# acerbilab/vbmc

Hardware: AMD Instinct MI355X
Metric: ELBO+grad evals/sec (Ns=1e4, K=50, D=10, N=400) (higher is better)
Workload: dtype f64; 1 GPU; BASELINE configs[2]: D=10 N=400 K=50 Ns=10000/component S=20, R=64 restarts batched per GPU per step, value+gradient, beta=0, no variance; restarts_per_gpu=64, parallelism=one GPU

## Files before the change

### vbmc_amd/csrc/entropy_mfma.h

```cpp
#pragma once
#include <type_traits>

#include "device_math.h"
#include "elbo_types.h"
#include "exp2_tab1k.h"
#include "logjoint_body.h"

typedef double mf4 __attribute__((ext_vector_type(4)));
struct EntTileAny { static constexpr bool rt = false, val = true; };
struct EntTileFull { static constexpr bool rt = false, val = false; };
struct EntTilePartial { static constexpr bool rt = false, val = true; };
#define VBMC_ENT_SPLIT(KT_, QS_, TL_, HV_) ((HV_) == 1)

#ifdef VBMC_INSTRUMENT
#define VBMC_DBG_WAVES 32768
__device__ unsigned long long g_ent_dbg[6 * VBMC_DBG_WAVES];
#endif

#define VBMC_STAG_FOR(KT_, QS_, TL_) ((KT_) == 1 || (KT_) == 4 || ((KT_) == 2 && (QS_) >= 6) || ((KT_) == 3 && (QS_) <= ((TL_) ? 5 : 8)))



constexpr bool ent_c2_for(int KT, int QS, int TL, int HV) {
  if (HV == 1) {
    if (KT == 2) return !(TL == 1 && QS >= 6);
    if (KT == 3) return QS <= 5 || (TL == 0 && QS != 7) || (TL == 1 && QS == 7);
    if (KT == 4) return QS >= 5;
    return true;
  }
  if (HV == 2) {
    if (KT == 2) return TL != 2;
    if (KT == 3) return !((TL == 1 && (QS == 5 || QS == 6)) || (TL == 2 && QS == 6));
    return true;
  }
  if (KT == 2) return !((TL == 1 && QS >= 6) || (TL == 2 && QS >= 5));
  if (KT == 3) return !(TL == 1 && QS == 7);
  return QS != 5;
}
constexpr bool ent_gp2_for(int KT, int QS, int TL, int HV) { return !(HV == 1 && KT == 1 && TL == 0 && QS <= 3); }

template <int HV>
__device__ __forceinline__ void ent_sync() {
  __builtin_amdgcn_fence(__ATOMIC_RELEASE, "wavefront");
  __builtin_amdgcn_wave_barrier();
  __builtin_amdgcn_fence(__ATOMIC_ACQUIRE, "wavefront");
}
template <int HV>
__device__ __forceinline__ void ent_sync_wg() {
  if (HV == 1) ent_sync<1>();
  else __syncthreads();
}

template <int QS, int KT, bool GRAD, bool SPARSE, int HV = 1, int TL = 0, bool CO = false, bool EM = true, bool WALK = false>
#define VBMC_ENT_EO(HV_) true
#define VBMC_ENT_ONE_WAVE(KT_, QS_, TL_, HV_) \
  (((HV_) == 1 && (KT_) == 4 && (QS_) >= 5) || ((HV_) == 1 && (KT_) == 3 && (QS_) >= 8) || ((HV_) == 4 && (KT_) == 4 && (QS_) >= 6) || \
   ((HV_) == 4 && (KT_) == 3 && (QS_) >= 9))
#define VBMC_ENT_WAVES(KT_, QS_, TL_, HV_) \
  (VBMC_ENT_ONE_WAVE(KT_, QS_, TL_, HV_) ? 1 : ((((KT_) <= 2 && (QS_) <= 4) && !((KT_) == 2 && (TL_) == 2 && (HV_) == 1)) ? 3 : 2))
__device__ __forceinline__ void ent_mfma_segment(const EntArgs& a, const int c, const int j, const int r, const int t0, const int t1,
                                                 const int pdone, const int ptot) {
  static_assert(!CO || (HV == 1 && QS <= 8 && !SPARSE), "the log-joint role exists for single-wave dense kernels at D <= 30");
  static_assert(!WALK || (HV == 1 && !CO), "the walk exists for single-wave workgroups without the log-joint role");
  static_assert(KT <= 4 && (HV == 1 || HV == 2 || HV == 4 || HV == 8), "larger mixtures are split over the waves of a workgroup (HV = 2, 4; round 5: 8, K <= 512)");
  static_assert(TL == 0 || ((TL == 1 || TL == 2) && !SPARSE), "the component tail (one or two values per lane) exists for the dense kernels only");
  constexpr int TLN = TL > 0 ? TL : 1;
  constexpr bool SP = SPARSE;
  constexpr int DP = 4 * QS;
  constexpr int NPV = (4 * QS + 15) / 16;
  constexpr int QL = QS;
  __shared__ double Et[16 * DP];
  constexpr bool GP2 = GRAD && ent_gp2_for(KT, QS, TL, HV);
  __shared__ double RQ_all[HV][GP2 ? 32 : 16];
  __shared__ double BND_all[HV][SPARSE ? KT * 16 * 3 : 1];
  constexpr int YXN = NPV * 4 * WAVE;
  constexpr bool EO = VBMC_ENT_EO(HV);
  constexpr bool YXSB = HV > 1 && EO;
  constexpr bool US = EO;
  constexpr bool VBL = GRAD && HV == 1 && (KT >= 3 || NPV >= 2);
  __shared__ double VBS_all[HV][VBL ? KT * 4 * NPV * WAVE : 1];
  constexpr bool C2 = EO && !SPARSE && ent_c2_for(KT, QS, TL, HV);
#define ENT_CI(kt_, rr_) (16 * (kt_) + 4 * (rr_) + lg)
  __shared__ __attribute__((aligned(16))) double SCP_all[HV][C2 ? KT * 16 * 2 : 2];
  __shared__ double BTL_all[HV][TL ? 4 * TL * DP : 1];
  constexpr bool NML = HV > 1 && EO;
  __shared__ double NMS_all[HV][NML ? KT * 4 * WAVE : 1];
#ifdef VBMC_INSTRUMENT
  const unsigned long long wckE = wall_clock64();
#endif
  int tid_ = threadIdx.x;
  if (WALK) asm volatile("" : "+v"(tid_));
  const int tid = tid_, wv = tid >> 6, hv = HV == 1 ? 0 : wv, lane = tid & 63;
  const int li = lane & 15, lg = lane >> 4;
  int D_ = a.D, K_ = a.K;
  const double *entp_ = a.entp, *vpd_ = a.vpd;
  double* part_ = a.part;
  if (WALK) asm volatile("" : "+s"(D_), "+s"(K_), "+s"(entp_), "+s"(vpd_), "+s"(part_));
  const int D = D_, K = K_;
  double* RQ = RQ_all[wv];
  double* NMS = NMS_all[wv];
  double* BND = BND_all[hv];
  double* VBS = VBS_all[hv];
  double* BTL = BTL_all[hv];
  double* SCP = SCP_all[hv];
  const int Kh = (K + HV - 1) / HV;
  const int kbase = hv * Kh;
  const int Kw = min(K, kbase + Kh) - kbase;
  const int PSg = D + ENTP_EXTRA;
  extern __shared__ double PB[];
  double* const TAB = PB;
  double* const YX = PB + VB_EXP_TAB1K_N;
  constexpr int NTH0 = WAVE * HV;
  constexpr int NTB0 = (VB_EXP_TAB1K_N + NTH0 - 1) / NTH0;
  double tt[NTB0];
#pragma unroll
  for (int u = 0; u < NTB0; ++u) tt[u] = c_exp2_tab1k[min(tid + u * NTH0, VB_EXP_TAB1K_N - 1)];
  const double sigj = vpd_[(size_t)r * VpLayout{D, K}.stride() + VpLayout{D, K}.sigma() + j];
  {
    const double* gsrc = entp_ + (size_t)r * K * PSg;
    constexpr int NT = WAVE * HV;
    const int n = K * PSg;
    int idx = tid;
    for (; idx + 7 * NT < n; idx += 8 * NT) {
      double t8[8];
#pragma unroll
      for (int u = 0; u < 8; ++u) t8[u] = gsrc[idx + u * NT];
#pragma unroll
      for (int u = 0; u < 8; ++u) PB[idx + u * NT] = t8[u];
    }
    {
      double t8[8];
#pragma unroll
      for (int u = 0; u < 8; ++u) t8[u] = (idx + u * NT < n) ? gsrc[idx + u * NT] : 0.0;
#pragma unroll
      for (int u = 0; u < 8; ++u) if (idx + u * NT < n) PB[idx + u * NT] = t8[u];
    }
  }
  __syncthreads();
  const double* gp = PB;
  const double* pj = gp + (size_t)j * PSg;
  const double cKj = pj[D + 1];
  const double hj_neg = 0.5 / (sigj * sigj);
  const int nr_last = TL ? 4 : max(1, min(4, (Kw - 16 * (KT - 1) + 3) >> 2));
  constexpr unsigned FULL_MASK = (1u << KT) - 1u;
  const double logwj = SPARSE ? log(pj[D + 2]) : 0.0;

  constexpr double ESC = VB_EXP_TAB1K_SCALE;
  double SA[KT][QL];
  double SC[KT];
  double VB[VBL ? 1 : KT][4][NPV];
  double WF[KT][4];
#pragma unroll
  for (int kt = 0; kt < KT; ++kt) {
    const int k = 16 * kt + li;
    const bool kv = k < Kw;
    const double* pk = gp + (size_t)(kv ? kbase + k : 0) * PSg;
    double h = pk[D];
    double m2 = 0.0;
    for (int d = 0; d < D; ++d) { double t = pk[d] - pj[d]; m2 = fma(t, t, m2); }
    if (SPARSE && lg == 0) {
      BND[(16 * kt + li) * 3 + 0] = sqrt(m2);
      BND[(16 * kt + li) * 3 + 1] = kv ? pk[D + 1] - cKj : -1.0e30;
      BND[(16 * kt + li) * 3 + 2] = h;
    }
#pragma unroll
    for (int q = 0; q < QL; ++q) {
      const int cc = 4 * q + lg;
      if (EO) {
        double sav = (kv && cc < D) ? ESC * (-2.0 * h * (pk[cc] - pj[cc])) : 0.0;
        if (C2) {
          if (cc == D) sav = kv ? ESC * (h + hj_neg) : 0.0;
          if (cc == D + 1) sav = ESC * (kv ? fma(h, m2, pk[D + 1]) - cKj : -1.0e6);
        }
        SA[kt][q] = sav;
      } else {
        double v;
        if (!kv) v = (cc == D + 1) ? -1.0e6 : 0.0;
        else if (cc < D) v = -2.0 * h * (pk[cc] - pj[cc]);
        else if (cc == D) v = h + hj_neg;
        else if (cc == D + 1) v = fma(h, m2, pk[D + 1]) - cKj;
        else v = 0.0;
        SA[kt][q] = ESC * v;
      }
    }
    SC[kt] = ESC * (!kv ? (lg == 1 ? -1.0e6 : 0.0)
                        : (lg == 0 ? h + hj_neg : (lg == 1 ? fma(h, m2, pk[D + 1]) - cKj : 0.0)));
    if (C2 && lg < 2) SCP[(16 * kt + li) * 2 + lg] = 2.0 * SC[kt];
#pragma unroll
    for (int rr = 0; rr < 4; ++rr) {
      const int k2 = ENT_CI(kt, rr);
      const bool kv2 = k2 < Kw;
      const double* p2 = gp + (size_t)(kv2 ? kbase + k2 : 0) * PSg;
      if (GRAD) {
#pragma unroll
        for (int pv = 0; pv < NPV; ++pv) {
          const int col = 16 * pv + li;
          double v = 0.0;
          if (kv2) {
            if (col == 0) v = p2[D + 2];
            else if (col == 1) v = p2[D + 3];
            else if (col < 2 + D) v = p2[D + 3] * (p2[col - 2] - pj[col - 2]);
          }
          if (VBL) VBS[((kt * 4 + rr) * NPV + pv) * WAVE + lane] = v;
          else VB[VBL ? 0 : kt][rr][pv] = v;
        }
      } else {
        WF[kt][rr] = kv2 ? p2[D + 2] : 0.0;
      }
    }
  }

  double tC0[TLN], tC1[TLN], VBt[TLN][NPV], WFt[TLN], Wt[TLN];
#pragma unroll
  for (int u = 0; u < TLN; ++u) {
    tC0[u] = 0.0; tC1[u] = 0.0; WFt[u] = 0.0; Wt[u] = 0.0;
#pragma unroll
    for (int pv = 0; pv < NPV; ++pv) VBt[u][pv] = 0.0;
  }
  if (TL) {
#pragma unroll
    for (int u = 0; u < TLN; ++u) {
      const int tq = 4 * u + lg;
      const int kq = 16 * KT + tq;
      const bool kvq = kq < Kw;
      const double* pq = gp + (size_t)(kvq ? kbase + kq : 0) * PSg;
      const double h = pq[D];
      double m2 = 0.0;
      for (int d = 0; d < D; ++d) { double t = pq[d] - pj[d]; m2 = fma(t, t, m2); }
      tC0[u] = kvq ? ESC * (h + hj_neg) : 0.0;
      tC1[u] = ESC * (kvq ? fma(h, m2, pq[D + 1]) - cKj : -1.0e6);
      for (int d = li; d < DP; d += 16) BTL[tq * DP + d] = (kvq && d < D) ? ESC * (-2.0 * h * (pq[d] - pj[d])) : 0.0;
      if (GRAD) {
#pragma unroll
        for (int pv = 0; pv < NPV; ++pv) {
          const int col = 16 * pv + li;
          double v = 0.0;
          if (kvq) {
            if (col == 0) v = pq[D + 2];
            else if (col == 1) v = pq[D + 3];
            else if (col < 2 + D) v = pq[D + 3] * (pq[col - 2] - pj[col - 2]);
          }
          VBt[u][pv] = v;
        }
      } else {
        WFt[u] = kvq ? pq[D + 2] : 0.0;
      }
    }
  }

  __syncthreads();
  {
#pragma unroll
    for (int u = 0; u < NTB0; ++u) if (VB_EXP_TAB1K_N % NTH0 == 0 || tid + u * NTH0 < VB_EXP_TAB1K_N) TAB[tid + u * NTH0] = tt[u];
  }
  __syncthreads();

#define SAV(kt_, q_) SA[kt_][q_]
  constexpr int VBR = (VBL && NPV == 1 && HV == 1 && KT == 3 && !CO) ? ((EM && QS <= 4) ? (TL == 2 ? 4 : 10) : 12) : 0;
  double VBreg[VBR > 0 ? VBR : 1];
#pragma unroll
  for (int u = 0; u < VBR; ++u) VBreg[u] = VBS[u * WAVE + lane];
#define VBV(kt_, rr_, pv_) (VBL ? (((kt_) * 4 + (rr_)) * NPV + (pv_) < VBR ? VBreg[(((kt_) * 4 + (rr_)) * NPV + (pv_)) < VBR ? (((kt_) * 4 + (rr_)) * NPV + (pv_)) : 0] : VBS[(((kt_) * 4 + (rr_)) * NPV + (pv_)) * WAVE + lane]) : VB[VBL ? 0 : (kt_)][rr_][pv_])
  double accH = 0.0, accG[NPV], accLG[NPV];
  double pm = 1.0;
  int pe = 0, pcnt = 0;
  double Wacc[KT][4];
#pragma unroll
  for (int pv = 0; pv < NPV; ++pv) { accG[pv] = 0.0; accLG[pv] = 0.0; }
#pragma unroll
  for (int kt = 0; kt < KT; ++kt)
#pragma unroll
    for (int rr = 0; rr < 4; ++rr) Wacc[kt][rr] = 0.0;

#ifdef VBMC_INSTRUMENT
  const unsigned long long wck0 = wall_clock64();
#endif
  const int ntile = (a.Mh + 15) >> 4;
  const double sfm0 = lg == 0 ? 1.0 : 0.0, sfm1 = lg == 1 ? 1.0 : 0.0;
  const int emask = (4 * (QS - 1) + lg < D) ? -1 : 0;
  const int emask2 = (QS >= 2 && 4 * (QS - 2) + lg < D) ? -1 : 0;
  const double* epsr = a.eps ? a.eps + (size_t)r * a.eps_stride_r + (size_t)j * a.Mh * D : nullptr;
  constexpr bool EPF = EM && HV == 1 && QS <= 4 && KT <= 3 && !SPARSE;
  double epre[EPF ? QS : 1];
  auto eps_fetch = [&](const int tile) {
#pragma unroll
    for (int u = 0; u < (EPF ? QS : 0); ++u) {
      const int idx = lane + u * WAVE, i = idx / DP, d = idx - i * DP;
      double v = 0.0;
      if (tile < t1 && d < D && tile * 16 + i < a.Mh) v = epsr[(size_t)(tile * 16 + i) * D + d];
      epre[u] = v;
    }
  };
  if (EPF && epsr) eps_fetch(t0);
  if (!epsr && (HV == 1 || hv == 0))
    for (int idx = lane; idx < 16 * DP; idx += WAVE) Et[idx] = 0.0;
  const int evm1 = emask, evm2 = emask2;
  const double c2u1 = (4 * (QS - 1) + lg == D) ? 1.0 : 0.0, c2o1 = (4 * (QS - 1) + lg == D + 1) ? 1.0 : 0.0;
  const double c2u2 = (QS >= 2 && 4 * (QS - 2) + lg == D) ? 1.0 : 0.0;

  auto tile_body = [&](const int tile, auto pkind) __attribute__((always_inline)) {
    using PK = decltype(pkind);
    const int b0 = tile * 16;
    ent_sync_wg<HV>();
    if (HV > 1 && hv != 0) {
    } else if (EPF && epsr) {
#pragma unroll
      for (int u = 0; u < (EPF ? QS : 0); ++u) Et[lane + u * WAVE] = US ? sigj * epre[u] : epre[u];
      eps_fetch(tile + 1);
    } else if (epsr) {
      for (int idx = lane; idx < 16 * DP; idx += WAVE) {
        const int i = idx / DP, d = idx - i * DP;
        Et[idx] = (d < D && b0 + i < a.Mh) ? (US ? sigj * epsr[(size_t)(b0 + i) * D + d] : epsr[(size_t)(b0 + i) * D + d]) : 0.0;
      }
    } else {
      unsigned long long seed_t = a.seed;
      if (WALK) asm volatile("" : "+s"(seed_t));
#pragma unroll
      for (int q = lg; q < QS; q += 4) {
        double z4[4] = {0.0, 0.0, 0.0, 0.0};
#define VBMC_RNG_CALL_FOR(KT_, QS_, TL_, HV_) ((HV_) == 2 && (((KT_) == 2 && (TL_) == 2 && (QS_) == 5) || ((KT_) == 3 && (TL_) == 0 && (QS_) == 7)))
        if constexpr (!VBMC_RNG_CALL_FOR(KT, QS, TL, HV)) {
        if (q < (D + 3) / 4) { const vb_d4 zz = vb_normal4i(seed_t, (unsigned)(b0 + li), (unsigned)j, (unsigned)(a.r0 + r * a.rstride), (unsigned)q); z4[0] = zz[0]; z4[1] = zz[1]; z4[2] = zz[2]; z4[3] = zz[3]; }
        } else {
        if (q < (D + 3) / 4) vb_normal4(seed_t, (unsigned)(b0 + li), (unsigned)j, (unsigned)(a.r0 + r * a.rstride), (unsigned)q, z4);
        }
#undef VBMC_RNG_CALL_FOR
        if (q < (D + 3) / 4) {
#pragma unroll
        for (int t = 0; t < 4; ++t) Et[li * DP + 4 * q + t] = US ? sigj * z4[t] : z4[t];
        }
      }
    }
    ent_sync_wg<HV>();
    double ev[QS];
    double e2 = 0.0;
#pragma unroll
    for (int q = 0; q < QS; ++q) {
      ev[q] = Et[li * DP + 4 * q + lg];
      if (q == QS - 1) ev[q] = __hiloint2double(__double2hiint(ev[q]) & evm1, __double2loint(ev[q]) & evm1);
      if (QS >= 2 && q == QS - 2) ev[q] = __hiloint2double(__double2hiint(ev[q]) & evm2, __double2loint(ev[q]) & evm2);
      e2 = fma(ev[q], ev[q], e2);
    }
    e2 = xor_sum16(e2);
    e2 = xor_sum32(e2);
    double shift = US ? fma(-e2, hj_neg, cKj) : cKj - 0.5 * e2;
    const double u2 = US ? e2 : sigj * sigj * e2;
    if (US && SPARSE) e2 *= 2.0 * hj_neg;
    constexpr bool partial = PK::val;
    const bool svalid = b0 + li < a.Mh;
    if (partial) shift = svalid ? shift : 0.0;
    unsigned act = FULL_MASK;
    if (SPARSE) {
      double e2m = e2;
      e2m = fmax(e2m, __shfl_xor(e2m, 1, 64)); e2m = fmax(e2m, __shfl_xor(e2m, 2, 64));
      e2m = fmax(e2m, __shfl_xor(e2m, 4, 64)); e2m = fmax(e2m, __shfl_xor(e2m, 8, 64));
      const double umax = sigj * sqrt(e2m);
      const double own = 0.5 * e2m - logwj;
      act = 0u;
#pragma unroll
      for (int kt = 0; kt < KT; ++kt) {
        const double* bk = BND + (16 * kt + li) * 3;
        const double t = fmax(0.0, bk[0] - umax);
        const double bnd = fma(bk[2] * t, t, bk[1]) + own;
        if (__any(bnd > -a.cutoff)) act |= 1u << kt;
      }
    }

    mf4 n[KT], nm[(EO && !NML) ? KT : 1];
    if (EO) {
      const double sfc = fma(u2, sfm0, sfm1);
      double sfl[QL];
#pragma unroll
      for (int q = 0; q < QL; ++q) sfl[q] = US ? ev[q] : ev[q] * sigj;
      if (C2) {
        sfl[QL - 1] = fma(u2, c2u1, sfl[QL - 1] + c2o1);
        if (QS >= 2) sfl[QL >= 2 ? QL - 2 : 0] = fma(u2, c2u2, sfl[QL >= 2 ? QL - 2 : 0]);
      }
#pragma unroll
      for (int kt = 0; kt < KT; ++kt) {
        n[kt] = (mf4){0.0, 0.0, 0.0, 0.0};
        if (!NML) nm[(EO && !NML) ? kt : 0] = (mf4){0.0, 0.0, 0.0, 0.0};
        if (C2) {
#pragma unroll
          for (int q = 0; q < QL; ++q) n[kt] = __builtin_amdgcn_mfma_f64_16x16x4f64(SAV(kt, q), sfl[q], n[kt], 0, 0, 0);
          mf4 e2nd;
#pragma unroll
          for (int rr = 0; rr < 4; ++rr) {
            const double2 pr = *reinterpret_cast<const double2*>(SCP + ENT_CI(kt, rr) * 2);
            e2nd[rr] = fma(pr.x, u2, pr.y) - n[kt][rr];
          }
          if (NML) {
#pragma unroll
            for (int rr = 0; rr < 4; ++rr) NMS[(kt * 4 + rr) * WAVE + lane] = e2nd[rr];
          } else {
            nm[(EO && !NML) ? kt : 0] = e2nd;
          }
        } else
        if (!SP || ((act >> kt) & 1u)) {
          const mf4 cacc = __builtin_amdgcn_mfma_f64_16x16x4f64(SC[kt], sfc, n[kt], 0, 0, 0);
          n[kt] = cacc;
#pragma unroll
          for (int q = 0; q < QL; ++q)
            n[kt] = __builtin_amdgcn_mfma_f64_16x16x4f64(SAV(kt, q), sfl[q], n[kt], 0, 0, 0);
          if (NML) {
            const mf4 e2nd = 2.0 * cacc - n[kt];
#pragma unroll
            for (int rr = 0; rr < 4; ++rr) NMS[(kt * 4 + rr) * WAVE + lane] = e2nd[rr];
          } else {
            nm[(EO && !NML) ? kt : 0] = 2.0 * cacc - n[kt];
          }
        }
      }
    }

    double ntl[TLN], ntm[TLN];
#pragma unroll
    for (int u = 0; u < TLN; ++u) { ntl[u] = 0.0; ntm[u] = 0.0; }
    if (TL) {
#pragma unroll
      for (int u = 0; u < TLN; ++u) {
        double lt = 0.0;
#pragma unroll
        for (int d = 0; d < DP; ++d) lt = fma(BTL[(4 * u + lg) * DP + d], Et[li * DP + d], lt);
        if (!US) lt *= sigj;
        const double ct = fma(tC0[u], u2, tC1[u]);
        ntl[u] = ct + lt;
        ntm[u] = ct - lt;
      }
    }

    auto exps = [&](mf4 (&x)[KT], auto k0c, auto k1c) {
      constexpr int k0 = decltype(k0c)::value, k1 = decltype(k1c)::value;
#pragma unroll
      for (int kt = k0; kt < k1; ++kt) {
        if (kt < KT - 1) {
          if (!SP || ((act >> kt) & 1u)) x[kt] = vb_exp_tab1k4<VB_EXP_TAB1K_QUAD>(x[kt], TAB);
          else x[kt] = (mf4){0.0, 0.0, 0.0, 0.0};
        } else if (SP && !((act >> (KT - 1)) & 1u)) {
          x[KT - 1] = (mf4){0.0, 0.0, 0.0, 0.0};
        } else if (nr_last == 4) {
          x[KT - 1] = vb_exp_tab1k4<VB_EXP_TAB1K_QUAD>(x[KT - 1], TAB);
        } else {
          mf4 t = x[KT - 1];
          x[KT - 1] = (mf4){0.0, 0.0, 0.0, 0.0};
          x[KT - 1][0] = vb_exp_tab1k<VB_EXP_TAB1K_QUAD>(t[0], TAB);
          if (nr_last > 1) x[KT - 1][1] = vb_exp_tab1k<VB_EXP_TAB1K_QUAD>(t[1], TAB);
          if (nr_last > 2) x[KT - 1][2] = vb_exp_tab1k<VB_EXP_TAB1K_QUAD>(t[2], TAB);
        }
      }
    };
    auto texp = [&](double (&t)[TLN]) {
      if (TL) {
#pragma unroll
        for (int u = 0; u < TLN; ++u) t[u] = vb_exp_tab1k<VB_EXP_TAB1K_QUAD>(t[u], TAB);
      }
    };
    auto pvstep = [&](mf4 (&x)[KT], mf4 (&Y)[NPV], int sg, const double (&tn)[TLN]) {
      constexpr bool TWO = NPV == 1 && KT <= 2;
      mf4 Y2s[TWO ? NPV : 1];
      mf4 (&Y2)[TWO ? NPV : 1] = Y2s;
#pragma unroll
      for (int pv = 0; pv < NPV; ++pv) { Y[pv] = (mf4){0.0, 0.0, 0.0, 0.0}; if (TWO) Y2[pv] = (mf4){0.0, 0.0, 0.0, 0.0}; }
#pragma unroll
      for (int kt = 0; kt < KT - 1; ++kt) {
        if (SP && !((act >> kt) & 1u)) continue;
#pragma unroll
        for (int pv = 0; pv < NPV; ++pv) {
          mf4& Yb = TWO ? Y2[TWO ? pv : 0] : Y[pv];
          Y[pv] = __builtin_amdgcn_mfma_f64_16x16x4f64(x[kt][0], VBV(kt, 0, pv), Y[pv], 0, 0, 0);
          Yb = __builtin_amdgcn_mfma_f64_16x16x4f64(x[kt][1], VBV(kt, 1, pv), Yb, 0, 0, 0);
          Y[pv] = __builtin_amdgcn_mfma_f64_16x16x4f64(x[kt][2], VBV(kt, 2, pv), Y[pv], 0, 0, 0);
          Yb = __builtin_amdgcn_mfma_f64_16x16x4f64(x[kt][3], VBV(kt, 3, pv), Yb, 0, 0, 0);
        }
      }
#pragma unroll
      for (int pv = 0; pv < NPV; ++pv) {
        mf4& Yb = TWO ? Y2[TWO ? pv : 0] : Y[pv];
        if (SP && !((act >> (KT - 1)) & 1u)) { if (TWO) Y[pv] += Yb; continue; }
        Y[pv] = __builtin_amdgcn_mfma_f64_16x16x4f64(x[KT - 1][0], VBV(KT - 1, 0, pv), Y[pv], 0, 0, 0);
        if (nr_last > 1) Yb = __builtin_amdgcn_mfma_f64_16x16x4f64(x[KT - 1][1], VBV(KT - 1, 1, pv), Yb, 0, 0, 0);
        if (nr_last > 2) Y[pv] = __builtin_amdgcn_mfma_f64_16x16x4f64(x[KT - 1][2], VBV(KT - 1, 2, pv), Y[pv], 0, 0, 0);
        if (nr_last > 3) Yb = __builtin_amdgcn_mfma_f64_16x16x4f64(x[KT - 1][3], VBV(KT - 1, 3, pv), Yb, 0, 0, 0);
        if (TL) {
#pragma unroll
          for (int u = 0; u < TLN; ++u) Y[pv] = __builtin_amdgcn_mfma_f64_16x16x4f64(tn[u], VBt[u][pv], Y[pv], 0, 0, 0);
        }
        if (TWO) Y[pv] += Yb;
      }
      if (HV > 1) {
        if (YXSB && sg == 1) __syncthreads();
#pragma unroll
        for (int pv = 0; pv < NPV; ++pv)
#pragma unroll
          for (int rr = 0; rr < 4; ++rr) YX[((YXSB ? 0 : sg) * HV + hv) * YXN + (pv * 4 + rr) * WAVE + lane] = Y[pv][rr];
        __syncthreads();
#pragma unroll
        for (int pv = 0; pv < NPV; ++pv)
#pragma unroll
          for (int rr = 0; rr < 4; ++rr) {
            double t = YX[((YXSB ? 0 : sg) * HV + 0) * YXN + (pv * 4 + rr) * WAVE + lane];
#pragma unroll
            for (int w = 1; w < HV; ++w) t += YX[((YXSB ? 0 : sg) * HV + w) * YXN + (pv * 4 + rr) * WAVE + lane];
            Y[pv][rr] = t;
          }
      }
    };
    auto put_q = [&](mf4 (&Y)[NPV]) {
      if (GP2 ? li < 2 : li == 0) {
#pragma unroll
        for (int rr = 0; rr < 4; ++rr) RQ[(GP2 ? 16 * li : 0) + lg + 4 * rr] = Y[0][rr];
      }
      ent_sync<HV>();
    };
    double arq = 0.0;
    constexpr bool TQ = GP2 && US && NPV == 1 && HV == 1 && EO && KT == 3 && QS <= 3 && !CO && !EM && VBMC_STAG_FOR(KT, QS, TL);
    double tq[TQ ? 4 : 1];
    auto get_rq = [&]() -> double {
      double qs_ = RQ[li];
      double rqs = vb_rcp(qs_);
      if (partial) {
        qs_ = svalid ? qs_ : 1.0;
        rqs = svalid ? rqs : 0.0;
      }
      if (GP2) arq = RQ[GP2 ? 16 + li : 0] * rqs;
      pm *= __builtin_amdgcn_frexp_mant(qs_);
      pe += __builtin_amdgcn_frexp_exp(qs_);
      accH += shift;
      return rqs;
    };
    auto wacc = [&](mf4 (&x)[KT], double rqs, const double (&tn)[TLN]) {
      if (TL) {
#pragma unroll
        for (int u = 0; u < TLN; ++u) Wt[u] = fma(tn[u], rqs, Wt[u]);
      }
#pragma unroll
      for (int kt = 0; kt < KT; ++kt) {
        if (SP && !((act >> kt) & 1u)) continue;
#pragma unroll
        for (int rr = 0; rr < 4; ++rr) Wacc[kt][rr] = fma(x[kt][rr], rqs, Wacc[kt][rr]);
      }
    };
    auto put_rq = [&](double rqs) {
      ent_sync<HV>();
      if (lg == 0) { RQ[li] = rqs; if (GP2) RQ[GP2 ? 16 + li : 0] = arq; }
      ent_sync<HV>();
    };
    auto gradpieces = [&](mf4 (&Y)[NPV], double ssig, auto sgc) {
      constexpr int SG = decltype(sgc)::value;
      if constexpr (GP2) {
#pragma unroll
        for (int rr = 0; rr < 4; ++rr) {
          const int i = lg + 4 * rr;
          const double rq = RQ[i], ar = RQ[GP2 ? 16 + i : 0];
#pragma unroll
          for (int pv = 0; pv < NPV; ++pv) {
            if (HV > 1 && (pv % HV) != hv) continue;
            const int d = min(max(16 * pv + li - 2, 0), DP - 1);
            double tv;
            if (TQ) { if (SG >= 0) tq[TQ ? rr : 0] = Et[i * DP + d]; tv = tq[TQ ? rr : 0]; }
            else tv = Et[i * DP + d];
            const double t = (US && SG > 0) ? tv : ((US && SG < 0) ? -tv : ssig * tv);
            const double gd = fma(t, ar, -(Y[pv][rr] * rq));
            accG[pv] += gd;
            accLG[pv] = fma(t, gd, accLG[pv]);
          }
        }
        ent_sync<HV>();
        return;
      }
      const int base = lane & 48;
#pragma unroll
      for (int rr = 0; rr < 4; ++rr) {
        const int i = lg + 4 * rr;
        const double Av = __shfl(Y[0][rr], base | 1, 64);
        const double rq = RQ[i];
#pragma unroll
        for (int pv = 0; pv < NPV; ++pv) {
          if (HV > 1 && (pv % HV) != hv) continue;
          const int d = 16 * pv + li - 2;
          if (d >= 0 && d < D) {
            const double t = (US && SG > 0) ? Et[i * DP + d] : ((US && SG < 0) ? -Et[i * DP + d] : ssig * Et[i * DP + d]);
            const double gd = (t * Av - Y[pv][rr]) * rq;
            accG[pv] += gd;
            accLG[pv] = fma(t, gd, accLG[pv]);
          }
        }
      }
      ent_sync<HV>();
    };
    auto fold = [&]() {
      if (++pcnt == 256) {
        pe += __builtin_amdgcn_frexp_exp(pm);
        pm = __builtin_amdgcn_frexp_mant(pm);
        pcnt = 0;
      }
    };
    using I0 = std::integral_constant<int, 0>;
    using IH = std::integral_constant<int, (KT + 1) / 2>;
    using IK = std::integral_constant<int, KT>;

    if constexpr (EO && GRAD && HV == 1 && VBMC_STAG_FOR(KT, QS, TL)) {
      mf4 Y[NPV];
      exps(n, I0{}, IK{});
      texp(ntl);
      pvstep(n, Y, 0, ntl);
      put_q(Y);
      exps(nm, I0{}, IH{});
      const double rqs = get_rq();
      put_rq(rqs);
      exps(nm, IH{}, IK{});
      texp(ntm);
      wacc(n, rqs, ntl);
      gradpieces(Y, sigj, std::integral_constant<int, 1>{});
      fold();
      pvstep(nm, Y, 1, ntm);
      put_q(Y);
      const double rqs2 = get_rq();
      wacc(nm, rqs2, ntm);
      put_rq(rqs2);
      gradpieces(Y, -sigj, std::integral_constant<int, -1>{});
      fold();
    } else {
      int sg = 0;
      double ssig = US ? 1.0 : sigj;
#pragma unroll 1
      for (;;) {
        if (!EO) {
          double sf[QS];
#pragma unroll
          for (int q = 0; q < QS; ++q) {
            const int cc = 4 * q + lg;
            constexpr bool EVREG = KT <= 3 && QS <= 7;
            sf[q] = (cc < D) ? ssig * (EVREG ? ev[q] : Et[li * DP + 4 * q + lg]) : ((cc == D) ? u2 : ((cc == D + 1) ? 1.0 : 0.0));
          }
#pragma unroll
          for (int kt = 0; kt < KT; ++kt) {
            n[kt] = (mf4){0.0, 0.0, 0.0, 0.0};
#pragma unroll
            for (int q = 0; q < QS; ++q) n[kt] = __builtin_amdgcn_mfma_f64_16x16x4f64(SA[kt][q], sf[q], n[kt], 0, 0, 0);
          }
        }
        exps(n, I0{}, IK{});
        texp(ntl);
        if (GRAD) {
          mf4 Y[NPV];
          pvstep(n, Y, sg, ntl);
          put_q(Y);
          const double rqs = get_rq();
          wacc(n, rqs, ntl);
          put_rq(rqs);
          gradpieces(Y, ssig, std::integral_constant<int, 0>{});
        } else {
          double qp = 0.0;
#pragma unroll
          for (int kt = 0; kt < KT; ++kt)
#pragma unroll
            for (int rr = 0; rr < 4; ++rr) qp = fma(WF[kt][rr], n[kt][rr], qp);
          if (TL) {
#pragma unroll
            for (int u = 0; u < TLN; ++u) qp = fma(WFt[u], ntl[u], qp);
          }
          qp += __shfl_xor(qp, 16, 64);
          qp += __shfl_xor(qp, 32, 64);
          if (HV > 1) {
            if (YXSB && sg == 1) __syncthreads();
            YX[((YXSB ? 0 : sg) * HV + hv) * YXN + lane] = qp;
            __syncthreads();
            qp = YX[((YXSB ? 0 : sg) * HV + 0) * YXN + lane];
#pragma unroll
            for (int w = 1; w < HV; ++w) qp += YX[((YXSB ? 0 : sg) * HV + w) * YXN + lane];
          }
          double qs_ = qp;
          if (partial) qs_ = svalid ? qp : 1.0;
          pm *= __builtin_amdgcn_frexp_mant(qs_);
          pe += __builtin_amdgcn_frexp_exp(qs_);
          accH += shift;
        }
        fold();
        if (sg) break;
        sg = 1;
        ssig = US ? -1.0 : -sigj;
        if (EO) {
#pragma unroll
          for (int kt = 0; kt < KT; ++kt) {
            if (NML) {
#pragma unroll
              for (int rr = 0; rr < 4; ++rr) n[kt][rr] = NMS[(kt * 4 + rr) * WAVE + lane];
            } else {
              n[kt] = nm[(EO && !NML) ? kt : 0];
            }
          }
        }
#pragma unroll
        for (int u = 0; u < TLN; ++u) ntl[u] = ntm[u];
      }
    }
  };
  if constexpr (VBMC_ENT_SPLIT(KT, QS, TL, HV)) {
    const int tf = min(t1, a.Mh >> 4);
    constexpr bool PRIO = CO ? QS <= 4 : VBMC_ENT_WAVES(KT, QS, TL, HV) > 1;
    const bool pr = PRIO && a.prio != 0;
    const int q1 = pr ? t0 + (ptot + 3) / 4 - pdone : -1, q2 = pr ? t0 + (ptot + 1) / 2 - pdone : -1, q3 = pr ? t0 + (3 * ptot + 3) / 4 - pdone : -1;
    if (pr && pdone == 0) __builtin_amdgcn_s_setprio(3);
    for (int tile = t0; tile < tf; ++tile) {
      if (tile == q1) __builtin_amdgcn_s_setprio(2);
      if (tile == q2) __builtin_amdgcn_s_setprio(1);
      if (tile == q3) __builtin_amdgcn_s_setprio(0);
      tile_body(tile, EntTileFull{});
    }
    if (tf < t1) tile_body(tf, EntTilePartial{});
  } else {
    for (int tile = t0; tile < t1; ++tile) tile_body(tile, EntTileAny{});
  }
#ifdef VBMC_INSTRUMENT
  const unsigned long long wck1 = wall_clock64();
#endif
  if (WALK) accH += vb_log_pos(pm, &pe) + 0.693147180559945309417 * (double)pe;
  else accH += log(pm) + 0.693147180559945309417 * (double)pe;
  if (lg != 0) accH = 0.0;

  double* o = part_ + (((size_t)r * K + j) * a.C + c) * a.ncol;
  accH = wave_sum(accH);
  if (lane == 0 && hv == 0) o[0] = accH;
  if (GRAD) {
    double sgsum = 0.0;
#pragma unroll
    for (int pv = 0; pv < NPV; ++pv) {
      double g = accG[pv], lgd = accLG[pv] / sigj;
      g += __shfl_xor(g, 16, 64); g += __shfl_xor(g, 32, 64);
      lgd += __shfl_xor(lgd, 16, 64); lgd += __shfl_xor(lgd, 32, 64);
      const int d = 16 * pv + li - 2;
      const bool dv = d >= 0 && d < D;
      const bool mine = HV == 1 || (pv % HV) == hv;
      if (dv && lg == 0 && mine) { o[1 + d] = g; o[2 + D + d] = lgd; }
      sgsum += (dv && lg == 0 && mine) ? lgd : 0.0;
    }
    sgsum = wave_sum(sgsum);
    if (HV > 1) {
      __syncthreads();
      if (lane == 0) YX[hv * YXN] = sgsum;
      __syncthreads();
      sgsum = YX[0];
#pragma unroll
      for (int w = 1; w < HV; ++w) sgsum += YX[w * YXN];
    }
    if (lane == 0 && hv == 0) o[1 + D] = sgsum;
#pragma unroll
    for (int kt = 0; kt < KT; ++kt)
#pragma unroll
      for (int rr = 0; rr < 4; ++rr) {
        double wv = Wacc[kt][rr];
        wv += __shfl_xor(wv, 1, 64); wv += __shfl_xor(wv, 2, 64);
        wv += __shfl_xor(wv, 4, 64); wv += __shfl_xor(wv, 8, 64);
        const int k = ENT_CI(kt, rr);
        if (li == 0 && k < Kw) o[2 + 2 * D + kbase + k] = wv;
      }
    if (TL) {
#pragma unroll
      for (int u = 0; u < TLN; ++u) {
        double wv = Wt[u];
        wv += __shfl_xor(wv, 1, 64); wv += __shfl_xor(wv, 2, 64);
        wv += __shfl_xor(wv, 4, 64); wv += __shfl_xor(wv, 8, 64);
        const int k = 16 * KT + 4 * u + lg;
        if (li == 0 && k < Kw) o[2 + 2 * D + kbase + k] = wv;
      }
    }
  }
#ifdef VBMC_INSTRUMENT
  if (lane == 0) {
    const size_t w = ((size_t)r * K + j) * a.C + c;
    if (w < VBMC_DBG_WAVES) {
      g_ent_dbg[6 * w + 0] = wckE; g_ent_dbg[6 * w + 1] = wck0; g_ent_dbg[6 * w + 2] = wck1; g_ent_dbg[6 * w + 3] = wall_clock64();
      g_ent_dbg[6 * w + 4] = __builtin_amdgcn_s_getreg(63492);
      g_ent_dbg[6 * w + 5] = __builtin_amdgcn_s_getreg(63508);
    }
  }
#endif
#undef VBV
#undef SAV
#undef ENT_CI
}

template <int QS, int KT, bool GRAD, bool SPARSE, int HV = 1, int TL = 0, bool CO = false, bool EM = true, bool WALK = false>
__global__ void __launch_bounds__(WAVE * HV, CO ? (QS <= 4 ? 2 : 1) : VBMC_ENT_WAVES(KT, QS, TL, HV)) k_entropy_mfma(EntArgs a) {
  const int ntile = (a.Mh + 15) >> 4;
  constexpr bool walk = WALK;
  int c = (int)blockIdx.x, j = CO ? (int)blockIdx.y - a.lj.rows : (int)blockIdx.y, r = (int)blockIdx.z;
  int tlo = ((int)blockIdx.x + a.c0) * a.tiles_per_chunk, thi = min(tlo + a.tiles_per_chunk, ntile), pdone = 0, rem = 0;
  if (!WALK && a.co_c2 > 0 && c >= a.co_c1) {
    tlo = a.co_c1 * a.tiles_per_chunk + (c - a.co_c1) * a.co_tpc2;
    thi = min(tlo + a.co_tpc2, ntile);
  }
  if (CO) {
    if ((int)blockIdx.y < a.lj.rows) {
      extern __shared__ double PB[];
      lj_co_role<4 * QS>(a.lj, a.vpd, PB);
      const int e = (int)(blockIdx.y * gridDim.x + blockIdx.x);
      if (a.co_c2 <= 0 || e >= a.K * a.co_c2) return;
      j = e / a.co_c2;
      c = a.co_c1 + (e - j * a.co_c2);
      tlo = a.co_c1 * a.tiles_per_chunk + (c - a.co_c1) * a.co_tpc2;
      thi = min(tlo + a.co_tpc2, ntile);
      __syncthreads();
    }
  }
  if (walk) {
    const int g = (int)blockIdx.x * a.walk_tpw;
    rem = min(a.walk_tpw, a.K * a.walk_R * ntile - g);
    const int p = g / ntile;
    tlo = g - p * ntile;
    r = p / a.K;
    j = p - r * a.K;
    c = (int)blockIdx.x - (g - tlo) / a.walk_tpw;
  }
  const int ptot = walk ? rem : thi - tlo;
  for (;;) {
    if (walk) thi = min(ntile, tlo + rem);
    ent_mfma_segment<QS, KT, GRAD, SPARSE, HV, TL, CO, EM, WALK>(a, c, j, r, tlo, thi, pdone, ptot);
    if (!walk) break;
    pdone += thi - tlo;
    rem -= thi - tlo;
    if (rem <= 0) break;
    if (++j == a.K) { j = 0; ++r; }
    tlo = 0;
    c = 0;
    __syncthreads();
  }
}
```

Measured before the change: 29840 evals/s.

## Transpose entropy gradient MFMA so per-sample sums stay in registers

For small-dimension single-wave gradient kernels, the weighted-value MFMA swaps its operands so that the result lands in a layout where each lane holds its own sample's q and weighted sums. The q and a-q terms are read directly from the accumulator registers, with a permlane32 swap, so the LDS round trip through RQ and its wave barriers go away. Gradient accumulation becomes per-dimension in a transposed layout, with a different final shuffle reduction. This adds extra registers and cross-lane swap ops and is gated by a hand-tuned table of (KT, QS, TL) configurations.

```diff
diff --git a/vbmc_amd/csrc/entropy_mfma.h b/vbmc_amd/csrc/entropy_mfma.h
--- a/vbmc_amd/csrc/entropy_mfma.h
+++ b/vbmc_amd/csrc/entropy_mfma.h
@@ -38,6 +38,13 @@
   return QS != 5;
 }
 constexpr bool ent_gp2_for(int KT, int QS, int TL, int HV) { return !(HV == 1 && KT == 1 && TL == 0 && QS <= 3); }
+constexpr bool ent_sl_for(int KT, int QS, int TL, int HV, bool GRAD, bool WALK) {
+  if (!(GRAD && HV == 1 && QS <= 3) || KT == 4 || WALK) return false;
+  if (QS == 3) return !((KT == 1 && TL == 0) || (KT == 2 && TL <= 1));
+  if (QS == 2) return KT == 3 || (KT == 2 && TL == 0);
+  return TL == 0 || (KT == 2 && TL == 1) || (KT == 3 && TL == 2);
+}
+constexpr bool ent_sl_evl_for(int KT, int QS, int TL) { return QS == 3 && KT == 3 && TL == 0; }
 
 template <int HV>
 __device__ __forceinline__ void ent_sync() {
@@ -70,8 +77,9 @@
   constexpr int NPV = (4 * QS + 15) / 16;
   constexpr int QL = QS;
   __shared__ double Et[16 * DP];
-  constexpr bool GP2 = GRAD && ent_gp2_for(KT, QS, TL, HV);
-  __shared__ double RQ_all[HV][GP2 ? 32 : 16];
+  constexpr bool SL = NPV == 1 && ent_sl_for(KT, QS, TL, HV, GRAD, WALK);
+  constexpr bool GP2 = GRAD && !SL && ent_gp2_for(KT, QS, TL, HV);
+  __shared__ double RQ_all[HV][SL ? 1 : (GP2 ? 32 : 16)];
   __shared__ double BND_all[HV][SPARSE ? KT * 16 * 3 : 1];
   constexpr int YXN = NPV * 4 * WAVE;
   constexpr bool EO = VBMC_ENT_EO(HV);
@@ -196,6 +204,13 @@
         for (int pv = 0; pv < NPV; ++pv) {
           const int col = 16 * pv + li;
           double v = 0.0;
+          if (SL) {
+            if (kv2) {
+              if (li >= 12) v = p2[D + 2];
+              else if (li >= 10) v = p2[D + 3];
+              else if (li < D) v = p2[D + 3] * (p2[li] - pj[li]);
+            }
+          } else
           if (kv2) {
             if (col == 0) v = p2[D + 2];
             else if (col == 1) v = p2[D + 3];
@@ -235,6 +250,13 @@
         for (int pv = 0; pv < NPV; ++pv) {
           const int col = 16 * pv + li;
           double v = 0.0;
+          if (SL) {
+            if (kvq) {
+              if (li >= 12) v = pq[D + 2];
+              else if (li >= 10) v = pq[D + 3];
+              else if (li < D) v = pq[D + 3] * (pq[li] - pj[li]);
+            }
+          } else
           if (kvq) {
             if (col == 0) v = pq[D + 2];
             else if (col == 1) v = pq[D + 3];
@@ -261,12 +283,13 @@
 #pragma unroll
   for (int u = 0; u < VBR; ++u) VBreg[u] = VBS[u * WAVE + lane];
 #define VBV(kt_, rr_, pv_) (VBL ? (((kt_) * 4 + (rr_)) * NPV + (pv_) < VBR ? VBreg[(((kt_) * 4 + (rr_)) * NPV + (pv_)) < VBR ? (((kt_) * 4 + (rr_)) * NPV + (pv_)) : 0] : VBS[(((kt_) * 4 + (rr_)) * NPV + (pv_)) * WAVE + lane]) : VB[VBL ? 0 : (kt_)][rr_][pv_])
-  double accH = 0.0, accG[NPV], accLG[NPV];
+  constexpr int NG = SL ? QS : NPV;
+  double accH = 0.0, accG[NG], accLG[NG];
   double pm = 1.0;
   int pe = 0, pcnt = 0;
   double Wacc[KT][4];
 #pragma unroll
-  for (int pv = 0; pv < NPV; ++pv) { accG[pv] = 0.0; accLG[pv] = 0.0; }
+  for (int pv = 0; pv < NG; ++pv) { accG[pv] = 0.0; accLG[pv] = 0.0; }
 #pragma unroll
   for (int kt = 0; kt < KT; ++kt)
 #pragma unroll
@@ -457,6 +480,9 @@
     };
     auto pvstep = [&](mf4 (&x)[KT], mf4 (&Y)[NPV], int sg, const double (&tn)[TLN]) {
       constexpr bool TWO = NPV == 1 && KT <= 2;
+      auto pvm = [&](double xa, double vb, mf4 acc) __attribute__((always_inline)) {
+        return SL ? __builtin_amdgcn_mfma_f64_16x16x4f64(vb, xa, acc, 0, 0, 0) : __builtin_amdgcn_mfma_f64_16x16x4f64(xa, vb, acc, 0, 0, 0);
+      };
       mf4 Y2s[TWO ? NPV : 1];
       mf4 (&Y2)[TWO ? NPV : 1] = Y2s;
 #pragma unroll
@@ -467,23 +493,23 @@
 #pragma unroll
         for (int pv = 0; pv < NPV; ++pv) {
           mf4& Yb = TWO ? Y2[TWO ? pv : 0] : Y[pv];
-          Y[pv] = __builtin_amdgcn_mfma_f64_16x16x4f64(x[kt][0], VBV(kt, 0, pv), Y[pv], 0, 0, 0);
-          Yb = __builtin_amdgcn_mfma_f64_16x16x4f64(x[kt][1], VBV(kt, 1, pv), Yb, 0, 0, 0);
-          Y[pv] = __builtin_amdgcn_mfma_f64_16x16x4f64(x[kt][2], VBV(kt, 2, pv), Y[pv], 0, 0, 0);
-          Yb = __builtin_amdgcn_mfma_f64_16x16x4f64(x[kt][3], VBV(kt, 3, pv), Yb, 0, 0, 0);
+          Y[pv] = pvm(x[kt][0], VBV(kt, 0, pv), Y[pv]);
+          Yb = pvm(x[kt][1], VBV(kt, 1, pv), Yb);
+          Y[pv] = pvm(x[kt][2], VBV(kt, 2, pv), Y[pv]);
+          Yb = pvm(x[kt][3], VBV(kt, 3, pv), Yb);
         }
       }
 #pragma unroll
       for (int pv = 0; pv < NPV; ++pv) {
         mf4& Yb = TWO ? Y2[TWO ? pv : 0] : Y[pv];
         if (SP && !((act >> (KT - 1)) & 1u)) { if (TWO) Y[pv] += Yb; continue; }
-        Y[pv] = __builtin_amdgcn_mfma_f64_16x16x4f64(x[KT - 1][0], VBV(KT - 1, 0, pv), Y[pv], 0, 0, 0);
-        if (nr_last > 1) Yb = __builtin_amdgcn_mfma_f64_16x16x4f64(x[KT - 1][1], VBV(KT - 1, 1, pv), Yb, 0, 0, 0);
-        if (nr_last > 2) Y[pv] = __builtin_amdgcn_mfma_f64_16x16x4f64(x[KT - 1][2], VBV(KT - 1, 2, pv), Y[pv], 0, 0, 0);
-        if (nr_last > 3) Yb = __builtin_amdgcn_mfma_f64_16x16x4f64(x[KT - 1][3], VBV(KT - 1, 3, pv), Yb, 0, 0, 0);
+        Y[pv] = pvm(x[KT - 1][0], VBV(KT - 1, 0, pv), Y[pv]);
+        if (nr_last > 1) Yb = pvm(x[KT - 1][1], VBV(KT - 1, 1, pv), Yb);
+        if (nr_last > 2) Y[pv] = pvm(x[KT - 1][2], VBV(KT - 1, 2, pv), Y[pv]);
+        if (nr_last > 3) Yb = pvm(x[KT - 1][3], VBV(KT - 1, 3, pv), Yb);
         if (TL) {
 #pragma unroll
-          for (int u = 0; u < TLN; ++u) Y[pv] = __builtin_amdgcn_mfma_f64_16x16x4f64(tn[u], VBt[u][pv], Y[pv], 0, 0, 0);
+          for (int u = 0; u < TLN; ++u) Y[pv] = pvm(tn[u], VBt[u][pv], Y[pv]);
         }
         if (TWO) Y[pv] += Yb;
       }
@@ -506,6 +532,7 @@
       }
     };
     auto put_q = [&](mf4 (&Y)[NPV]) {
+      if constexpr (SL) return;
       if (GP2 ? li < 2 : li == 0) {
 #pragma unroll
         for (int rr = 0; rr < 4; ++rr) RQ[(GP2 ? 16 * li : 0) + lg + 4 * rr] = Y[0][rr];
@@ -515,14 +542,20 @@
     double arq = 0.0;
     constexpr bool TQ = GP2 && US && NPV == 1 && HV == 1 && EO && KT == 3 && QS <= 3 && !CO && !EM && VBMC_STAG_FOR(KT, QS, TL);
     double tq[TQ ? 4 : 1];
-    auto get_rq = [&]() -> double {
-      double qs_ = RQ[li];
+    auto get_rq = [&](mf4 (&Y)[NPV]) -> double {
+      double qs_ = SL ? Y[0][3] : RQ[li];
       double rqs = vb_rcp(qs_);
       if (partial) {
         qs_ = svalid ? qs_ : 1.0;
         rqs = svalid ? rqs : 0.0;
       }
       if (GP2) arq = RQ[GP2 ? 16 + li : 0] * rqs;
+      if (SL) {
+        const double t = Y[0][2] * rqs;
+        const auto lo = __builtin_amdgcn_permlane32_swap((unsigned)__double2loint(t), (unsigned)__double2loint(t), false, false);
+        const auto hi = __builtin_amdgcn_permlane32_swap((unsigned)__double2hiint(t), (unsigned)__double2hiint(t), false, false);
+        arq = __hiloint2double((int)hi[1], (int)lo[1]);
+      }
       pm *= __builtin_amdgcn_frexp_mant(qs_);
       pe += __builtin_amdgcn_frexp_exp(qs_);
       accH += shift;
@@ -541,12 +574,27 @@
       }
     };
     auto put_rq = [&](double rqs) {
+      if constexpr (SL) return;
       ent_sync<HV>();
       if (lg == 0) { RQ[li] = rqs; if (GP2) RQ[GP2 ? 16 + li : 0] = arq; }
       ent_sync<HV>();
     };
-    auto gradpieces = [&](mf4 (&Y)[NPV], double ssig, auto sgc) {
+    auto gradpieces = [&](mf4 (&Y)[NPV], double rqs, double ssig, auto sgc) {
       constexpr int SG = decltype(sgc)::value;
+      constexpr bool EVL = SL && ent_sl_evl_for(KT, QS, TL);
+      int eo = li * DP + lg;
+      if (EVL) asm volatile("" : "+v"(eo));
+      if constexpr (SL) {
+#pragma unroll
+        for (int r = 0; r < QS; ++r) {
+          const double tv = EVL ? Et[eo + 4 * r] : ev[r];
+          const double t = (US && SG > 0) ? tv : ((US && SG < 0) ? -tv : ssig * tv);
+          const double gd = fma(t, arq, -(Y[0][r] * rqs));
+          accG[r] += gd;
+          accLG[r] = fma(t, gd, accLG[r]);
+        }
+        return;
+      }
       if constexpr (GP2) {
 #pragma unroll
         for (int rr = 0; rr < 4; ++rr) {
@@ -606,19 +654,19 @@
       pvstep(n, Y, 0, ntl);
       put_q(Y);
       exps(nm, I0{}, IH{});
-      const double rqs = get_rq();
+      const double rqs = get_rq(Y);
       put_rq(rqs);
       exps(nm, IH{}, IK{});
       texp(ntm);
       wacc(n, rqs, ntl);
-      gradpieces(Y, sigj, std::integral_constant<int, 1>{});
+      gradpieces(Y, rqs, sigj, std::integral_constant<int, 1>{});
       fold();
       pvstep(nm, Y, 1, ntm);
       put_q(Y);
-      const double rqs2 = get_rq();
+      const double rqs2 = get_rq(Y);
       wacc(nm, rqs2, ntm);
       put_rq(rqs2);
-      gradpieces(Y, -sigj, std::integral_constant<int, -1>{});
+      gradpieces(Y, rqs2, -sigj, std::integral_constant<int, -1>{});
       fold();
     } else {
       int sg = 0;
@@ -646,10 +694,10 @@
           mf4 Y[NPV];
           pvstep(n, Y, sg, ntl);
           put_q(Y);
-          const double rqs = get_rq();
+          const double rqs = get_rq(Y);
           wacc(n, rqs, ntl);
           put_rq(rqs);
-          gradpieces(Y, ssig, std::integral_constant<int, 0>{});
+          gradpieces(Y, rqs, ssig, std::integral_constant<int, 0>{});
         } else {
           double qp = 0.0;
 #pragma unroll
@@ -724,6 +772,20 @@
   if (lane == 0 && hv == 0) o[0] = accH;
   if (GRAD) {
     double sgsum = 0.0;
+    if constexpr (SL) {
+#pragma unroll
+      for (int r = 0; r < QS; ++r) {
+        double g = accG[r], lgd = accLG[r] / sigj;
+        g += __shfl_xor(g, 1, 64); g += __shfl_xor(g, 2, 64);
+        g += __shfl_xor(g, 4, 64); g += __shfl_xor(g, 8, 64);
+        lgd += __shfl_xor(lgd, 1, 64); lgd += __shfl_xor(lgd, 2, 64);
+        lgd += __shfl_xor(lgd, 4, 64); lgd += __shfl_xor(lgd, 8, 64);
+        const int d = 4 * r + lg;
+        const bool dv = li == 0 && d < D;
+        if (dv) { o[1 + d] = g; o[2 + D + d] = lgd; }
+        sgsum += dv ? lgd : 0.0;
+      }
+    } else {
 #pragma unroll
     for (int pv = 0; pv < NPV; ++pv) {
       double g = accG[pv], lgd = accLG[pv] / sigj;
@@ -734,6 +796,7 @@
       const bool mine = HV == 1 || (pv % HV) == hv;
       if (dv && lg == 0 && mine) { o[1 + d] = g; o[2 + D + d] = lgd; }
       sgsum += (dv && lg == 0 && mine) ? lgd : 0.0;
+    }
     }
     sgsum = wave_sum(sgsum);
     if (HV > 1) {
```

After: 31060 evals/s, median of 6. +4.1%, better.
